# LCJebe/PCReg

Hardware: AMD Instinct MI355X
Metric: KNN Gpairs/s end-to-end (search + filters + RANSAC per step; registrations/s = 1000/ms_per_step) (higher is better)
Workload: dtype f32 (search: f16-split matrix-core candidates, exact f32 re-rank) / f64 (RANSAC)

## Files before the change

include/pcreg.h:

```cpp
#ifndef PCREG_H
#define PCREG_H
#include <stddef.h>
#include <stdint.h>

#ifdef __cplusplus
extern "C" {
#endif

#define PCREG_OK            0
#define PCREG_E_ARG         1
#define PCREG_E_HIP         2
#define PCREG_E_NODEVICE    3
#define PCREG_E_WORKSPACE   4

#define PCREG_KNN_MAX_K 32

#define PCREG_METRIC_SAD 0
#define PCREG_METRIC_SSD 1

typedef struct pcreg_ransac_opts {
    int32_t  minPtNum;
    int32_t  iterNum;
    double   thDist;
    double   thInlrRatio;
// ... 4 lines not shown

typedef struct pcreg_match_opts {
    int32_t metric;
    double  matchThreshold;
    double  maxRatio;
    int32_t unique;
    int32_t prenormalized;
    int32_t unnormalize;
    double  norm_factor;
    int32_t change_metric;
    double  metric_factor;
} pcreg_match_opts;

const char* pcreg_last_error(void);
const char* pcreg_version(void);
int  pcreg_device_count(int* count);
int  pcreg_set_device(int ordinal);
int  pcreg_device_name(char* buf, int cap);
int  pcreg_debug_set(const char* key, int value);
int  pcreg_debug_match_stats(long long out[8], int reset);
int  pcreg_debug_knn_stats(long long out[4], int reset);
int  pcreg_debug_knn_unit_stats(long long out[2], int reset);
int  pcreg_debug_ransac_stats(long long out[3], int reset);
int  pcreg_debug_cluster_stats(long long out[4], int reset);


int pcreg_estimate_transform(const double* pts1, const double* pts2, int n, int ld,
                             double T[16], int* empty);

int pcreg_calc_dists(const double T[16], const double* pts1, const double* pts2, int n, int ld,
                     double* d);

int pcreg_ransac(const double* pts1, const double* pts2, int n, int ld,
                 const pcreg_ransac_opts* opts, const int32_t* sample_idx,
                 double T[16], int32_t* inlier_idx, int* n_inliers, int* num_success,
                 int* max_inliers, int* failed, int32_t* iter_inl, int32_t* iter_inl_ref);

int pcreg_ransac_batched(const double* pts1, const double* pts2, int total, int ld,
                         const int32_t* offsets, int B, const pcreg_ransac_opts* opts,
                         const int32_t* sample_idx, double* T, int32_t* inlier_idx,
                         int32_t* n_inliers, int32_t* num_success, int32_t* max_inliers,
                         int32_t* failed);

int pcreg_knn2_points_f32(const float* q, int Q, int ldq, const float* m, int M, int ldm,
                          int32_t* idx, float* dist);

// ... 319 lines not shown
```

pcreg_amd/_lib.py:

```python
from __future__ import annotations

import ctypes as C
import os

_HERE = os.path.dirname(os.path.abspath(__file__))
LIB_PATH = os.environ.get("PCREG_LIB") or os.path.join(_HERE, "libpcreg_hip.so")

PCREG_OK, PCREG_E_ARG, PCREG_E_HIP, PCREG_E_NODEVICE, PCREG_E_WORKSPACE = 0, 1, 2, 3, 4
KNN_MAX_K = 32
METRIC_SAD, METRIC_SSD = 0, 1
LAYOUT_FEATURE_MAJOR, LAYOUT_ROW_MAJOR = 0, 1


class PcregError(RuntimeError):
    def __init__(self, code: int, msg: str):
        super().__init__(f"libpcreg_hip error {code}: {msg}")
        self.code = code


class RansacOpts(C.Structure):
    _fields_ = [("minPtNum", C.c_int32), ("iterNum", C.c_int32), ("thDist", C.c_double),
                ("thInlrRatio", C.c_double), ("REFINE", C.c_int32), ("VERBOSE", C.c_int32),
                ("seed", C.c_uint64)]


class MatchOpts(C.Structure):
    _fields_ = [("metric", C.c_int32), ("matchThreshold", C.c_double), ("maxRatio", C.c_double),
                ("unique", C.c_int32), ("prenormalized", C.c_int32), ("unnormalize", C.c_int32),
                ("norm_factor", C.c_double), ("change_metric", C.c_int32), ("metric_factor", C.c_double)]


class DescOpts(C.Structure):
    _fields_ = [("min_pts", C.c_int32), ("max_pts", C.c_int32), ("R", C.c_double), ("thVar", C.c_double * 2),
                ("k", C.c_double), ("ALIGN_POINTS", C.c_int32)]


class DevRansacResult(C.Structure):
    _fields_ = [("T", C.c_double * 16), ("n_inliers", C.c_int32), ("num_success", C.c_int32),
                ("max_inliers", C.c_int32), ("failed", C.c_int32), ("n", C.c_int32), ("winner", C.c_int32)]


SYMBOLS = [
    "pcreg_last_error", "pcreg_version", "pcreg_device_count", "pcreg_set_device", "pcreg_device_name", "pcreg_debug_set", "pcreg_debug_match_stats",
    "pcreg_debug_knn_stats", "pcreg_debug_knn_unit_stats", "pcreg_debug_ransac_stats", "pcreg_debug_cluster_stats", "pcreg_debug_dev_model_export", "pcreg_debug_search_export",
    "pcreg_estimate_transform", "pcreg_calc_dists", "pcreg_ransac", "pcreg_ransac_batched",
    "pcreg_knn2_points_f32", "pcreg_match_points_f32", "pcreg_match_features", "pcreg_get_matches", "pcreg_desc_set_create", "pcreg_desc_set_destroy", "pcreg_desc_set_size", "pcreg_get_matches_on_sets", "pcreg_get_matches_segmented_on_sets", "pcreg_sphere_counts", "pcreg_sphere_sweep", "pcreg_sphere_model_create", "pcreg_sphere_model_destroy", "pcreg_sphere_sweep_on_model", "pcreg_final_stage_limits", "pcreg_final_stage", "pcreg_get_matches_segmented", "pcreg_get_local_points",
    "pcreg_model_create", "pcreg_model_destroy", "pcreg_model_size", "pcreg_model_match_points_f32", "pcreg_model_knn_f32", "pcreg_knn_points_f32",
    "pcreg_model_range_f32", "pcreg_range_points_f32", "pcreg_model_cluster_f32", "pcreg_cluster_points_f32",
    "pcreg_dev_model_create", "pcreg_dev_model_destroy", "pcreg_dev_model_search_workspace", "pcreg_dev_model_search_f32",
    "pcreg_dev_model_knn_workspace", "pcreg_dev_model_knn_f32", "pcreg_dev_merge_topk_f32",
    "pcreg_dev_model_range_workspace", "pcreg_dev_model_range_count_f32", "pcreg_dev_model_range_fill_f32",
    "pcreg_dev_model_cluster_workspace", "pcreg_dev_model_cluster_f32",
    "pcreg_model_score_f32", "pcreg_dev_model_score_workspace", "pcreg_dev_model_score_f32",
    "pcreg_model_refit_f32", "pcreg_dev_model_refit_workspace", "pcreg_dev_model_refit_f32",
    "pcreg_model_normals_f32", "pcreg_point_normals_f32", "pcreg_dev_model_normals_workspace", "pcreg_dev_model_normals_f32",
    "pcreg_model_refit_plane_f32", "pcreg_dev_model_refit_plane_workspace", "pcreg_dev_model_refit_plane_f32",
    "pcreg_unique_rows3", "pcreg_aggregate_matches", "pcreg_dev_unique_rows3_workspace", "pcreg_dev_unique_rows3_f64",
    "pcreg_dev_aggregate_matches_workspace", "pcreg_dev_aggregate_matches", "pcreg_dev_estimate_transform_indexed",
    "pcreg_dev_model_match_f32", "pcreg_dev_model_match_table_f32", "pcreg_dev_match_from_table_f32",
    "pcreg_align_points_knn", "pcreg_align_points_knn_f32", "pcreg_align_points_knn_batched", "pcreg_spatial_histogram_descriptors",
    "pcreg_spatial_histogram_descriptors_f32", "pcreg_spatial_histogram_descriptors_mixed",
    "pcreg_dev_knn2_points_f32_workspace", "pcreg_dev_knn2_points_f32", "pcreg_dev_merge_top2_f32", "pcreg_dev_merge_top2_strided_f32",
    "pcreg_dev_ransac_workspace", "pcreg_dev_ransac",
    "pcreg_dev_ransac_partial", "pcreg_dev_ransac_finish", "pcreg_dev_ransac_finish_parts",
    "pcreg_dev_search_kernel_timing", "pcreg_dev_search_kernel_ms",
    "pcreg_dev_spatial_histogram_descriptors_workspace", "pcreg_dev_spatial_histogram_descriptors",
    "pcreg_dev_spatial_histogram_descriptors_rows_u16", "pcreg_dev_get_matches_rows_u16",
# ... 59 lines not shown
            vp, i, f = C.c_void_p, C.c_int, C.c_float
            L.pcreg_dev_model_refit_f32.argtypes = [vp, vp, i, i, vp, i, f, vp, vp, vp, vp, vp, vp, C.c_size_t, vp]
            L.pcreg_model_refit_f32.argtypes = [vp, vp, i, i, vp, i, f, i, vp, vp, vp, vp]
        if hasattr(L, "pcreg_dev_model_normals_workspace"):
            L.pcreg_dev_model_normals_workspace.restype = C.c_size_t
            L.pcreg_dev_model_normals_workspace.argtypes = [C.c_int] * 2
            vp, i = C.c_void_p, C.c_int
            L.pcreg_dev_model_normals_f32.argtypes = [vp, i, vp, vp, i, vp, vp, C.c_size_t, vp]
            L.pcreg_model_normals_f32.argtypes = [vp, i, vp, vp, i, vp]
            L.pcreg_point_normals_f32.argtypes = [vp, i, i, i, vp, vp, i, vp]
        if hasattr(L, "pcreg_dev_model_refit_plane_workspace"):
            L.pcreg_dev_model_refit_plane_workspace.restype = C.c_size_t
            L.pcreg_dev_model_refit_plane_workspace.argtypes = [C.c_int] * 3
            vp, i, f = C.c_void_p, C.c_int, C.c_float
            L.pcreg_dev_model_refit_plane_f32.argtypes = [vp, vp, i, i, vp, i, f, vp, i, vp, vp, vp, vp, vp, vp, vp, vp, C.c_size_t, vp]
            L.pcreg_model_refit_plane_f32.argtypes = [vp, vp, i, i, vp, i, f, i, vp, i, i, vp, vp, vp, vp, vp, vp]
        if hasattr(L, "pcreg_dev_unique_rows3_workspace"):
            for name in ("pcreg_dev_unique_rows3_workspace", "pcreg_dev_aggregate_matches_workspace"):
                getattr(L, name).restype = C.c_size_t
                getattr(L, name).argtypes = [C.c_int]
        for name, args in (("pcreg_debug_knn_stats", [C.POINTER(C.c_longlong), C.c_int]),
                           ("pcreg_debug_knn_unit_stats", [C.POINTER(C.c_longlong), C.c_int]),
                           ("pcreg_debug_ransac_stats", [C.POINTER(C.c_longlong), C.c_int]),
                           ("pcreg_debug_dev_model_export", [C.c_void_p] * 4 + [C.POINTER(C.c_float), C.c_void_p]),
                           ("pcreg_debug_search_export", [C.c_void_p, C.c_size_t, C.c_int, C.c_int] + [C.c_void_p] * 3)):
            if hasattr(L, name):
                getattr(L, name).argtypes = args
        _lib = L
    return _lib


def check(rc: int) -> None:
    if rc != PCREG_OK:
        raise PcregError(rc, lib().pcreg_last_error().decode(errors="replace"))
```

pcreg_amd/csrc/api.hip:

```cpp
#include "common.hpp"
#include <atomic>
#include <cstdarg>
#include <cmath>
#include <mutex>
#include <algorithm>
#include <vector>

namespace pcreg {

static thread_local char g_err[512] = "no error";
void set_error(const char* fmt, ...) {
    va_list ap; va_start(ap, fmt);
    vsnprintf(g_err, sizeof g_err, fmt, ap);
    va_end(ap);
}

constexpr int kKnnMaxK = PCREG_KNN_MAX_K;
constexpr int kKnnMaxQ = 4 << 20;
constexpr int kRangeMaxQ = 4 << 20;
constexpr int kScoreMaxQ = 4 << 20;
static std::mutex g_mu;
static int g_device_ok = -1;
static hipStream_t g_stream = nullptr;

// ... 30 lines not shown
        size[slot] = want;
    }
    *out = ptr[slot];
    return PCREG_OK;
}
void Scratch::release_all() {
    for (int i = 0; i < kSlots; ++i) if (ptr[i]) { (void)hipFree(ptr[i]); ptr[i] = nullptr; size[i] = 0; }
}
Scratch& scratch() { static Scratch s; return s; }

}

using namespace pcreg;

#define GUARD()                                                     \
    std::lock_guard<std::mutex> lock__(g_mu);                       \
    do { int rc__ = ensure_device(); if (rc__) return rc__; } while (0)
#define TRY(expr) do { int rc__ = (expr); if (rc__) return rc__; } while (0)

namespace pcreg {
static std::atomic<int> g_debug[kDbgCount];
int debug_flag(DebugKey k) { return g_debug[k].load(std::memory_order_relaxed); }
struct Counters { DebugKey key; int n; unsigned long long* dev; };
static Counters g_match_stats{kDbgMatchStats, 8, nullptr}, g_knn_stats{kDbgKnnStats, 6, nullptr}, g_ransac_stats{kDbgRansacStats, 3, nullptr},
                g_cluster_stats{kDbgClusterStats, 4, nullptr};
static unsigned long long* counters_dev(Counters& c) {
    if (!debug_flag(c.key)) return nullptr;
    if (!c.dev) {
        if (hipMalloc((void**)&c.dev, c.n * sizeof(unsigned long long)) != hipSuccess) { c.dev = nullptr; return nullptr; }
        (void)hipMemset(c.dev, 0, c.n * sizeof(unsigned long long));
    }
    return c.dev;
}
static int counters_read(const Counters& c, long long* out, int reset, int first = 0, int count = -1) {
    PCREG_ARG(out != nullptr);
    if (count < 0) count = c.n - first;
    for (int k = 0; k < count; ++k) out[k] = 0;
    if (!c.dev) return PCREG_OK;
    PCREG_HIP(hipDeviceSynchronize());
    unsigned long long h[8];
    PCREG_HIP(hipMemcpy(h, c.dev + first, count * sizeof h[0], hipMemcpyDeviceToHost));
    for (int k = 0; k < count; ++k) out[k] = (long long)h[k];
    if (reset) PCREG_HIP(hipMemset(c.dev + first, 0, count * sizeof h[0]));
    return PCREG_OK;
}
unsigned long long* match_stats_dev() { return counters_dev(g_match_stats); }
unsigned long long* knn_stats_dev() { return counters_dev(g_knn_stats); }
unsigned long long* ransac_stats_dev() { return counters_dev(g_ransac_stats); }
unsigned long long* cluster_stats_dev() { return counters_dev(g_cluster_stats); }
}

extern "C" {

int pcreg_debug_set(const char* key, int value) {
    static const char* const names[pcreg::kDbgCount] = {"knn_exact", "match_exact", "match_force_fallback", "ransac_fused", "ransac_nolane",
                                                        "ransac_f64score", "ransac_resident_f64", "align_times", "align_shape", "seg_debug",
                                                        "seg_batched", "seg_wave_finalize", "match_stats", "final_batch_mb", "knn_nocull",
                                                        "knn_stats", "ransac_pass2", "ransac_stats", "range_sort_cap", "cluster_noskip",
                                                        "cluster_stats", "knn_tail_cap", "score_batch_slots"};
    PCREG_ARG(key != nullptr);
    for (int k = 0; k < pcreg::kDbgCount; ++k)
        if (!strcmp(key, names[k])) { pcreg::g_debug[k].store(value, std::memory_order_relaxed); return PCREG_OK; }
    pcreg::set_error("pcreg_debug_set: unknown key '%s'", key);
    return PCREG_E_ARG;
}

int pcreg_debug_match_stats(long long out[8], int reset) { return pcreg::counters_read(pcreg::g_match_stats, out, reset); }
int pcreg_debug_knn_stats(long long out[4], int reset) { return pcreg::counters_read(pcreg::g_knn_stats, out, reset, 0, 4); }
int pcreg_debug_knn_unit_stats(long long out[2], int reset) { return pcreg::counters_read(pcreg::g_knn_stats, out, reset, 4, 2); }
int pcreg_debug_ransac_stats(long long out[3], int reset) { return pcreg::counters_read(pcreg::g_ransac_stats, out, reset); }
int pcreg_debug_cluster_stats(long long out[4], int reset) { return pcreg::counters_read(pcreg::g_cluster_stats, out, reset); }

const char* pcreg_last_error(void) { return g_err; }
const char* pcreg_version(void) { return "pcreg-hip 0.1 (gfx950)"; }

int pcreg_device_count(int* count) {
    PCREG_ARG(count != nullptr);
    hipError_t e = hipGetDeviceCount(count);
    if (e != hipSuccess) { *count = 0; (void)hipGetLastError(); }
    return PCREG_OK;
}

static void*  g_pin[2] = {nullptr, nullptr};
static size_t g_pin_bytes[2] = {0, 0};
static hipEvent_t g_pairs_ev = nullptr;

int pcreg_set_device(int ordinal) {
    std::lock_guard<std::mutex> lock(g_mu);
    int count = 0;
    if (hipGetDeviceCount(&count) != hipSuccess || count <= 0) { set_error("no HIP device available"); (void)hipGetLastError(); return PCREG_E_NODEVICE; }
    PCREG_ARG(ordinal >= 0 && ordinal < count);
    scratch().release_all();
    if (g_stream) { (void)hipStreamDestroy(g_stream); g_stream = nullptr; }
// ... 1855 lines not shown
```

pcreg_amd/csrc/common.hpp:

```cpp
#pragma once
#include <cstdlib>
#include <hip/hip_runtime.h>
#include <cstdint>
#include <cstdio>
#include <cstring>
#include <algorithm>
#include <string>
#include "../../include/pcreg.h"

namespace pcreg {

void set_error(const char* fmt, ...);
int  ensure_device();

#define PCREG_HIP(call)                                                                  \
    do {                                                                                 \
        hipError_t e__ = (call);                                                         \
        if (e__ != hipSuccess) {                                                         \
            ::pcreg::set_error("%s failed: %s (%s:%d)", #call, hipGetErrorString(e__),   \
                               __FILE__, __LINE__);                                      \
            return PCREG_E_HIP;                                                          \
        }                                                                                \
    } while (0)

// ... 28 lines not shown
    kDbgKnnExact = 0,
    kDbgMatchExact,
    kDbgMatchForceFallback,
    kDbgRansacFused,
    kDbgRansacNoLane,
    kDbgRansacF64Score,
    kDbgRansacResidentF64,
    kDbgAlignTimes,
    kDbgAlignShape,
    kDbgSegDebug,
    kDbgSegBatched,
    kDbgSegWaveFinalize,
    kDbgMatchStats,
    kDbgFinalBatchMB,
    kDbgKnnNoCull,
    kDbgKnnStats,
    kDbgRansacPass2,
    kDbgRansacStats,
    kDbgRangeSortCap,
    kDbgClusterNoSkip,
    kDbgClusterStats,
    kDbgKnnTailCap,
    kDbgScoreBatchSlots,
    kDbgCount
};
int debug_flag(DebugKey k);
unsigned long long* match_stats_dev();
unsigned long long* knn_stats_dev();
unsigned long long* ransac_stats_dev();
unsigned long long* cluster_stats_dev();
#ifdef PCREG_EXPERIMENTS
static inline int pcreg_env_int(const char* name, int dflt) { const char* e = getenv(name); return e ? atoi(e) : dflt; }
static inline const char* pcreg_env_str(const char* name) { return getenv(name); }
#define PCREG_EXP_ENV(name, dflt) pcreg_env_int(name, dflt)
#define PCREG_EXP_STR(name) pcreg_env_str(name)
#else
#define PCREG_EXP_ENV(name, dflt) (dflt)
#define PCREG_EXP_STR(name) ((const char*)nullptr)
#endif

static inline size_t align_up(size_t x, size_t a) { return (x + a - 1) / a * a; }

struct WsWalk {
    char* base; size_t off = 0;
    explicit WsWalk(void* b) : base((char*)b) {}
    void* take_bytes(size_t bytes) { void* p = base ? base + off : nullptr; off += bytes; return p; }
// ... 169 lines not shown
```

pcreg_amd/csrc/ransac.hip:

```cpp
#include "common.hpp"
#include "moments.hpp"
#include <cfloat>
#include <cstddef>
#include <cstdio>
#include <cstdlib>

namespace pcreg {
namespace {

constexpr int kBlock = 256;
constexpr int kWavesPerBlock = 4;
constexpr int HB = 4;

struct RansacArgs {
    const double* p1; const double* p2; int ld;
    const int32_t* offsets;
    const int32_t* n_dev;
    int n_cap; int iters; int m;
    double thDist; double ratio; int refine; unsigned long long seed;
    const int32_t* sample_idx;
    int hpw;
    int hyp0g;
    double* TF;
    int32_t* cnt1; int32_t* cnt2; unsigned char* has;
// ... 892 lines not shown
    double* T1; unsigned char* v1; unsigned char* pass1; unsigned char* v2;
    unsigned char* cert;
    double* certq;
    double* bounds;
    void* sel_ctr;
    double* bpart;
    int n_rec_blocks;
    double* mom;
    int32_t* part;
    int pb;
    unsigned long long* masks;
    int nslots_cap;
    double* rec;
    double* mpart;
    uint4* dig;
    int32_t* pass_list;
    int32_t* n_pass;
    unsigned char* dense;
    int use_lane;
    float* c32;
    int n32;
    float* T32a; float* T32b;
    int use_f32;
    float* p32;
    int32_t* perm;
    unsigned char* bkt;
    void* bctr;
};

__device__ __forceinline__ int staged_n(const RansacArgs& a) { return min(a.n_dev ? *a.n_dev : a.n_cap, a.n_cap); }
__device__ __forceinline__ void staged_origin(const StagedArgs& sa, double (&o)[6]) {
#pragma unroll
    for (int c = 0; c < 6; ++c) o[c] = sa.bounds[4 + c];
}

__device__ __forceinline__ void rs_records_body(const StagedArgs& sa, int block) {
    const RansacArgs& a = sa.a;
    const int n = staged_n(a);
    const int i = block * 256 + threadIdx.x;
    double m1 = 0.0, m2 = 0.0, c1m = 0.0, c2m = 0.0;
    double o[6] = {0.0, 0.0, 0.0, 0.0, 0.0, 0.0}, g2[2] = {0.0, 0.0};
    if (n >= 1) {
        const Pts<false> P0{a.p1, a.p2, a.ld, nullptr, n};
        ransac_origin(P0, n, o, g2);
        g2[0] *= kGridReach * kGridReach; g2[1] *= kGridReach * kGridReach;
        if (block == 0 && threadIdx.x < 8) {
// ... 227 lines not shown
            for (int s = 0; s < kSS; ++s) {
                const unsigned long long b = __ballot((sqdist(q[s], T) < th) & act[s]);
                cnt += __popcll(b);
                if (EMIT) {
                    asm volatile("v_writelane_b32 %0, %1, %2" : "+v"(mine_lo) : "s"((int)(unsigned)b), "n"(s));
                    asm volatile("v_writelane_b32 %0, %1, %2" : "+v"(mine_hi) : "s"((int)(unsigned)(b >> 32)), "n"(s));
                }
            }
            if (lane == 0) s_cnt[wave][h - h0] += cnt;
            if (EMIT && lane < kSS)
                sa.masks[(size_t)h * sa.nslots_cap + (size_t)pb * (kSPts / 64) + wave * kSS + lane] =
                    ((unsigned long long)(unsigned)mine_hi << 32) | (unsigned)mine_lo;
        }
    }
    __syncthreads();
    for (int hl = threadIdx.x; hl < h1 - h0; hl += kSW * 64) {
        int c = 0;
#pragma unroll
        for (int w = 0; w < kSW; ++w) c += s_cnt[w][hl];
        sa.part[(size_t)blockIdx.x * a.iters + h0 + hl] = c;
    }
}

__device__ __forceinline__ void make_t32(const double (&T)[12], const double (&o)[6], double A, double B, double th,
                                         float* __restrict__ out , const bool resident = false ) {
    const double u = 5.9604644775390625e-08;
    double rho = 0.0, tau = 0.0;
#pragma unroll
    for (int r = 0; r < 3; ++r) {
        const double tp = T[r * 4 + 3] + (T[r * 4] * o[3] + T[r * 4 + 1] * o[4] + T[r * 4 + 2] * o[5]) - o[r];
        rho = fmax(rho, sqrt(T[r * 4] * T[r * 4] + T[r * 4 + 1] * T[r * 4 + 1] + T[r * 4 + 2] * T[r * 4 + 2]));
        tau = fmax(tau, fabs(tp));
        out[r * 3] = (float)T[r * 4]; out[r * 3 + 1] = (float)T[r * 4 + 1]; out[r * 3 + 2] = (float)T[r * 4 + 2];
        out[9 + r] = (float)tp;
    }
    const double e1 = resident ? 6.1 * u * (A + B * rho + tau) : u * (A + 5.1 * (B * rho + tau));
    const double E = 1.5 * (2.0 * 1.7320508075688774 * sqrt(4.0 * th) * e1 + 3.0 * e1 * e1 + 5.2 * u * 4.0 * th);
    float lo = -INFINITY, hi = INFINITY;
    if (E == E && E <= 0.5 * th && th > 0.0 && tau < 1e30 && A < 1e15 && B < 1e15) {
        lo = (float)(th - E); if ((double)lo > th - E) lo = nextafterf(lo, -INFINITY);
        hi = (float)(th + E); if ((double)hi < th + E) hi = nextafterf(hi, INFINITY);
    }
    out[12] = lo; out[13] = hi; out[14] = 0.0f; out[15] = 0.0f;
}

__device__ __forceinline__ void rs_fold_maxima(const StagedArgs& sa, double (&mx)[4]) {
    __shared__ double s_mx[4][4];
#pragma unroll
    for (int k = 0; k < 4; ++k) mx[k] = 0.0;
    for (int b = threadIdx.x; b < sa.n_rec_blocks; b += 256) {
#pragma unroll
        for (int k = 0; k < 4; ++k) mx[k] = fmax(mx[k], sa.bpart[(size_t)b * 4 + k]);
    }
#pragma unroll
    for (int k = 0; k < 4; ++k) {
#pragma unroll
        for (int o_ = 32; o_ > 0; o_ >>= 1) mx[k] = fmax(mx[k], __shfl_xor(mx[k], o_));
    }
    if ((threadIdx.x & 63) == 0) {
#pragma unroll
        for (int k = 0; k < 4; ++k) s_mx[threadIdx.x >> 6][k] = mx[k];
    }
    __syncthreads();
#pragma unroll
    for (int k = 0; k < 4; ++k) mx[k] = fmax(fmax(s_mx[0][k], s_mx[1][k]), fmax(s_mx[2][k], s_mx[3][k]));
}
__device__ __forceinline__ void rs_digits_body(const StagedArgs& sa, uint4* __restrict__ dig, int block, const double (&bounds)[4]);
__global__ __launch_bounds__(256) void rs_stage2_kernel(StagedArgs sa, const double* __restrict__ TT, float* __restrict__ out, int n_t32,
                                                        uint4* __restrict__ dig) {
    const RansacArgs& a = sa.a;
    double mx[4];
    rs_fold_maxima(sa, mx);
    if ((int)blockIdx.x >= n_t32) { rs_digits_body(sa, dig, blockIdx.x - n_t32, mx); return; }
    if (blockIdx.x == 0 && threadIdx.x < 4) sa.bounds[threadIdx.x] = mx[threadIdx.x];
    const int h = blockIdx.x * blockDim.x + threadIdx.x;
    if (h >= a.iters || !sa.use_f32) return;
    const int n = staged_n(a);
    if (n < 1) return;
    double o[6]; staged_origin(sa, o);
    double T[12];
#pragma unroll
    for (int k = 0; k < 12; ++k) T[k] = TT[(size_t)h * 12 + k];
    make_t32(T, o, sqrt(mx[2]) * (1.0 + 1e-12), sqrt(mx[3]) * (1.0 + 1e-12), a.thDist, out + (size_t)h * 16);
}

__device__ __forceinline__ float sqdist32(const float (&p)[6], const float (&T)[12]) {
    const float tx = __builtin_fmaf(p[3], T[0], __builtin_fmaf(p[4], T[1], __builtin_fmaf(p[5], T[2], T[9])));
    const float ty = __builtin_fmaf(p[3], T[3], __builtin_fmaf(p[4], T[4], __builtin_fmaf(p[5], T[5], T[10])));
    const float tz = __builtin_fmaf(p[3], T[6], __builtin_fmaf(p[4], T[7], __builtin_fmaf(p[5], T[8], T[11])));
    const float dx = p[0] - tx, dy = p[1] - ty, dz = p[2] - tz;
    return __builtin_fmaf(dz, dz, __builtin_fmaf(dy, dy, dx * dx));
}

typedef int rs_i32x16 __attribute__((ext_vector_type(16)));
template <bool EMIT>
__global__ __launch_bounds__(kSW * 64) void rs_score32_kernel(StagedArgs sa, const double* __restrict__ TT,
                                                              const float* __restrict__ T32,
                                                              const unsigned char* __restrict__ valid,
                                                              int32_t* __restrict__ acc ) {
    const RansacArgs& a = sa.a;
    __shared__ int s_cnt[kSW][kSChunk];
    const int n = staged_n(a);
    const int lane = threadIdx.x & 63, wave = __builtin_amdgcn_readfirstlane(threadIdx.x >> 6);
    const int h0 = blockIdx.y * kSChunk, h1 = min(a.iters, h0 + kSChunk);
    const double th = a.thDist;
    for (int hl = threadIdx.x; hl < kSW * kSChunk; hl += kSW * 64) (&s_cnt[0][0])[hl] = 0;
    unsigned long long vmask[(kSChunk + 63) / 64];
#pragma unroll
    for (int k = 0; k < (kSChunk + 63) / 64; ++k) {
        const int h = h0 + k * 64 + lane;
        vmask[k] = __ballot(h < h1 && k * 64 + lane < kSChunk && valid[h] != 0);
    }
    __syncthreads();
    for (int pb = blockIdx.x; pb * kSPts < n; pb += gridDim.x) {
        float q[kSS][6];
        const int ibase = pb * kSPts + wave * kSS * 64 + lane;
#pragma unroll
        for (int s = 0; s < kSS; ++s) {
            const int i = ibase + s * 64;
            const bool act = i < n;
            const int ii = act ? i : 0;
#pragma unroll
            for (int c = 0; c < 6; ++c) q[s][c] = sa.c32[(size_t)c * sa.n32 + ii];
            if (!act) q[s][0] = __builtin_nanf("");
        }
        rs_i32x16 RA, RB;
#define PCREG_ROW_LOAD(R, H) { const float* rp_ = T32 + (size_t)min((H), h1 - 1) * 16; asm volatile("s_load_dwordx16 %0, %1, 0x0" : "=&s"(R) : "s"(rp_)); }
#define PCREG_ROW_WAIT(R) asm volatile("s_waitcnt lgkmcnt(0)" : "+s"(R))
#define PCREG_SCORE_HYP(H, R)                                                                                      \
        if ((vmask[((H) - h0) >> 6] >> (((H) - h0) & 63)) & 1ull) {                                \
            float T[12];                                                                                           \
            _Pragma("unroll") for (int k = 0; k < 12; ++k) { const int w_ = R[k]; T[k] = __int_as_float(w_); }                 \
            const int wlo_ = R[12], whi_ = R[13]; const float thlo = __int_as_float(wlo_), thhi = __int_as_float(whi_);          \
            unsigned long long b[kSS], band = 0ull;                                                                \
            _Pragma("unroll") for (int s = 0; s < kSS; ++s) {                                                      \
                const float d = sqdist32(q[s], T);                                                                 \
                b[s] = __ballot(d < thlo);                                                                         \
                band |= __ballot(d <= thhi) ^ b[s];       \
            }                                                                                                      \
            if (band != 0ull) {       \
                double T64[12];       \
                _Pragma("unroll") for (int k = 0; k < 12; ++k) T64[k] = TT[(size_t)(H) * 12 + k];    \
                _Pragma("unroll 1") for (int s = 0; s < kSS; ++s) {       \
                    const int i = ibase + s * 64;                         \
                    const bool act = i < n;                                                                        \
                    const int ii = act ? i : 0;                                                                    \
                    float qq[6];                                                                                   \
                    _Pragma("unroll") for (int c = 0; c < 6; ++c) qq[c] = sa.c32[(size_t)c * sa.n32 + ii];         \
                    if (!act) qq[0] = __builtin_nanf("");                                                          \
                    const float d = sqdist32(qq, T);                                                               \
                    if ((__ballot(d <= thhi) ^ __ballot(d < thlo)) != 0ull) {                     \
                        double p[6];                                                                               \
                        _Pragma("unroll") for (int c = 0; c < 3; ++c) { p[c] = a.p1[ii + (size_t)c * a.ld]; p[3 + c] = a.p2[ii + (size_t)c * a.ld]; } \
// ... 1033 lines not shown
                for (int e = 0; e < 15; ++e) mom[e] += pp[e];
            }
            v2 = fit_moments(c1, mom, o, T2, true);
        } else if (c1 == 3) {
#pragma unroll
            for (int e = 0; e < 27; ++e) mom[e] = sa.mom[(size_t)h * 27 + e];
            double A1[3][3], A2[3][3];
#pragma unroll
            for (int j = 0; j < 3; ++j)
#pragma unroll
                for (int c = 0; c < 3; ++c) { A1[j][c] = mom[j * 6 + c]; A2[j][c] = mom[j * 6 + 3 + c]; }
            v2 = fit_3pt(A1, A2, T2);
        } else {
#pragma unroll
            for (int e = 0; e < 27; ++e) mom[e] = sa.mom[(size_t)h * 27 + e];
            v2 = fit_moments(c1, mom, o, T2, sa.cert[h] != 0);
        }
    }
#pragma unroll
    for (int k = 0; k < 12; ++k) a.TF[(size_t)h * 12 + k] = T2[k];
    sa.v2[h] = v2;
    if (sa.use_f32 && v2) {
        double o32[6]; staged_origin(sa, o32);
        make_t32(T2, o32, sqrt(sa.bounds[2]) * (1.0 + 1e-12), sqrt(sa.bounds[3]) * (1.0 + 1e-12), a.thDist, sa.T32b + (size_t)h * 16);
    }
}

template <int NTHR>
__device__ void ransac_emit_result(const RansacArgs& a, int n, int off, pcreg_dev_ransac_result* r, int32_t* inlier_idx,
                                   bool failed, const double* s_T , int ns, int maxInl, int winner,
                                   int* s_base, int* s_wcnt) {
    const int lane = threadIdx.x & 63, wave = threadIdx.x >> 6;
    if (threadIdx.x == 0) *s_base = 0;
    __syncthreads();
    if (threadIdx.x < 16) {
        int k = threadIdx.x & 3, j = threadIdx.x >> 2;
        double v = 0.0;
        if (!failed) v = (j < 3) ? s_T[j * 4 + k] : (k == 3 ? 1.0 : 0.0);
        r->T[k + 4 * j] = v;
    }
    if (threadIdx.x == 0) {
        r->failed = failed; r->num_success = failed ? 0 : ns; r->max_inliers = failed ? 0 : maxInl;
        r->n = n; r->winner = winner;
    }
    if (failed) { if (threadIdx.x == 0) r->n_inliers = 0; return; }
    double T[12];
#pragma unroll
// ... 520 lines not shown
    s.cnt1 = w.take<int32_t>(h); s.cnt2 = w.take<int32_t>(h);
    s.has = w.take<unsigned char>(h); s.msc = w.take<double>(h * 16);
    sa.T1 = w.take<double>(h * 12); sa.mom = w.take<double>(h * 27);
    sa.part = w.take<int32_t>(h * kSMaxPB);
    sa.v1 = w.take<unsigned char>(h); sa.pass1 = w.take<unsigned char>(h); sa.v2 = w.take<unsigned char>(h);
    sa.cert = w.take<unsigned char>(h); sa.dense = w.take<unsigned char>(h);
    sa.bounds = (double*)w.take_bytes(256);
    sa.n_rec_blocks = (int)((slots * 64 + 255) / 256);
    sa.bpart = w.take<double>((size_t)sa.n_rec_blocks * 4);
    sa.sel_ctr = w.take_bytes(512);
    sa.certq = w.take<double>(h * 2);
    if (nc >= kStagedMinN) {
        sa.nslots_cap = (int)slots;
        sa.masks = w.take<unsigned long long>(h * slots);
        sa.rec = w.take<double>(slots * 64 * kRec + 32);
        sa.mpart = w.take<double>(staged_chunks_cap(nc) * h * 15);
        sa.pass_list = w.take<int32_t>(h);
        sa.dig = w.take<uint4>(slots * 2 * 256);
        sa.n_pass = (int32_t*)w.take_bytes(256);
        sa.n32 = (int)slots * 64;
        sa.c32 = w.take<float>((size_t)sa.n32 * 6);
        sa.T32a = w.take<float>(h * 16); sa.T32b = w.take<float>(h * 16);
        sa.p32 = w.take<float>((size_t)sa.n32 * 6);
        sa.perm = w.take<int32_t>((size_t)sa.n32);
        sa.bkt = w.take<unsigned char>((size_t)sa.n32);
        sa.bctr = w.take_bytes(align_up(sizeof(BCtr), 256));
    }
    *bytes = w.bytes(); return s;
}
size_t ransac_workspace_bytes(int iters, int B, int n_cap) { size_t b; (void)ransac_ws_layout(iters, B, n_cap, nullptr, &b); return b; }

constexpr int kHyp32NClasses = 2;
constexpr int kHyp32Classes[kHyp32NClasses] = {1024, 2048};
constexpr int kHyp32Waves[kHyp32NClasses] = {8, 16};
constexpr int kHyp32BatchCap = 3242;
static size_t hyp32_lds_bytes(int n, int nw) { return (size_t)((n + 127) / 128 * 128) * 72 + ((size_t)nw * 4 + 6) * sizeof(double); }
template <int NW>
static int launch_hyp32(const RansacArgs& a, dim3 grid, size_t lds, hipStream_t st) {
    static bool attr_set = false;
    if (!attr_set) {
        PCREG_HIP(hipFuncSetAttribute((const void*)ransac_hyp32_kernel<NW, true>, hipFuncAttributeMaxDynamicSharedMemorySize, 160 * 1024));
        PCREG_HIP(hipFuncSetAttribute((const void*)ransac_hyp32_kernel<NW, false>, hipFuncAttributeMaxDynamicSharedMemorySize, 160 * 1024));
        attr_set = true;
    }
    if (a.refine) hipLaunchKernelGGL((ransac_hyp32_kernel<NW, true>), grid, dim3(NW * 64), lds, st, a);
    else hipLaunchKernelGGL((ransac_hyp32_kernel<NW, false>), grid, dim3(NW * 64), lds, st, a);
// ... 28 lines not shown
        hipLaunchKernelGGL(ransac_hyp_kernel, dim3((o.iterNum + pb4 - 1) / pb4, B), dim3(kBlock), lds, st, a);
    } else if (n_cap > 0 && n_cap <= (offsets ? kHyp32BatchCap : kHyp32Classes[kHyp32NClasses - 1])) {
        int hpw = 64;
        while (hpw > 8 && total / hpw < 256LL * 4 * 2) hpw >>= 1;
        a.hpw = hpw;
        a.msc = lay.msc;
        const int c = n_cap <= kHyp32Classes[0] ? 0 : 1;
        a.n_lo = -1; a.n_hi = std::min(n_cap, kHyp32Classes[c]);
        const int nw = kHyp32Waves[c], per_block = hpw * nw;
        const dim3 grid((o.iterNum + per_block - 1) / per_block, B);
        const int rc = nw == 8 ? launch_hyp32<8>(a, grid, hyp32_lds_bytes(a.n_hi, nw), st) : launch_hyp32<16>(a, grid, hyp32_lds_bytes(a.n_hi, nw), st);
        if (rc != PCREG_OK) return rc;
        const int lo = a.n_hi;
        if (n_cap > lo) {
            a.n_lo = lo; a.n_hi = -1;
            const int pb4 = hpw * kWavesPerBlock;
            hipLaunchKernelGGL(ransac_hyp_kernel, dim3((o.iterNum + pb4 - 1) / pb4, B), dim3(kBlock), 0, st, a);
        }
    } else if (B == 1 && !offsets && staged_pays(n_cap, o.iterNum) && !debug_flag(kDbgRansacFused)) {
        StagedArgs sa = lay.sa;
        sel_ctr = sa.sel_ctr;
        sa.use_lane = a.refine && !debug_flag(kDbgRansacNoLane);
        sa.use_f32 = !debug_flag(kDbgRansacF64Score);
        int pb = (n_cap + kSPts - 1) / kSPts; if (pb > kSMaxPB) pb = kSMaxPB; if (pb < 1) pb = 1;
        sa.pb = pb;
        int hpw = (int)((total + 250LL * kTW - 1) / (250LL * kTW));
        if (hpw < 1) hpw = 1;
        if (hpw > 16) hpw = 16;
        a.hpw = hpw;
        sa.a = a;
        const int it = o.iterNum;
        const dim3 sgrid(pb, (it + kSChunk - 1) / kSChunk);
        const int n_fit = (it + 255) / 256;
        hipLaunchKernelGGL(rs_stage1_kernel, dim3((unsigned)(n_fit + sa.n_rec_blocks)), dim3(256), 0, st, sa, n_fit);
        const int n_t32 = (it + 255) / 256, n_dig = sa.use_lane ? (int)staged_slots_cap(n_cap) * 2 : 0;
        hipLaunchKernelGGL(rs_stage2_kernel, dim3((unsigned)(n_t32 + n_dig)), dim3(256), 0, st, sa, (const double*)sa.T1, sa.T32a, n_t32, sa.dig);
        if (sa.use_f32) {
            if (sa.use_lane)
                hipLaunchKernelGGL(rs_score32_kernel<true>, sgrid, dim3(kSW * 64), 0, st, sa, (const double*)sa.T1, (const float*)sa.T32a, (const unsigned char*)sa.v1, (int32_t*)nullptr);
            else
                hipLaunchKernelGGL(rs_score32_kernel<false>, sgrid, dim3(kSW * 64), 0, st, sa, (const double*)sa.T1, (const float*)sa.T32a, (const unsigned char*)sa.v1, (int32_t*)nullptr);
        } else if (sa.use_lane) {
            hipLaunchKernelGGL(rs_score_kernel<true>, sgrid, dim3(kSW * 64), 0, st, sa, (const double*)sa.T1, (const unsigned char*)sa.v1);
        } else {
            hipLaunchKernelGGL(rs_score_kernel<false>, sgrid, dim3(kSW * 64), 0, st, sa, (const double*)sa.T1, (const unsigned char*)sa.v1);
        }
        hipLaunchKernelGGL(rs_pass1_kernel, dim3((it + 255) / 256), dim3(256), 0, st, sa);
        if (a.refine) {
            if (sa.use_lane)
                hipLaunchKernelGGL(rs_moments_mfma_kernel, dim3((it + kMmWaves * kMmRows - 1) / (kMmWaves * kMmRows), (unsigned)staged_chunks_cap(n_cap)), dim3(kMmWaves * 64), 0, st, sa,
                                   (const uint4*)sa.dig, (const unsigned long long*)sa.masks);
            hipLaunchKernelGGL(rs_moments_kernel, dim3((it + hpw * kTW - 1) / (hpw * kTW)), dim3(kTBlock), 0, st, sa);
            hipLaunchKernelGGL(rs_fit2_kernel, dim3((it + 63) / 64), dim3(64), 0, st, sa);
            fold_finish = !part && n_cap <= kSelBlocks * kSelPerThread * kSelThreads;
            const int p2mode = debug_flag(kDbgRansacPass2);
            const bool bounded = fold_finish && sa.use_f32 && !iter_inl_ref && p2mode != 1 && (p2mode == 2 || bounded_pays(n_cap, it));
            if (bounded) {
                const int S = std::min(kBSeeds, it), nbc = (n_cap + kBBlk - 1) / kBBlk;
                const int n_seed_wg = (S * nbc + 3) / 4, n_ord_wg = (n_cap + 255) / 256;
// ... 132 lines not shown
```

Before: 122,200.

## Add slot-level certification to skip per-point RANSAC scoring behind debug flag

```diff
diff --git a/include/pcreg.h b/include/pcreg.h
--- a/include/pcreg.h
+++ b/include/pcreg.h
@@ -50,6 +50,7 @@
 int  pcreg_debug_knn_stats(long long out[4], int reset);
 int  pcreg_debug_knn_unit_stats(long long out[2], int reset);
 int  pcreg_debug_ransac_stats(long long out[3], int reset);
+int  pcreg_debug_ransac_slot_stats(long long out[2], int reset);
 int  pcreg_debug_cluster_stats(long long out[4], int reset);
 
 
diff --git a/pcreg_amd/_lib.py b/pcreg_amd/_lib.py
--- a/pcreg_amd/_lib.py
+++ b/pcreg_amd/_lib.py
@@ -42,7 +42,7 @@
 
 SYMBOLS = [
     "pcreg_last_error", "pcreg_version", "pcreg_device_count", "pcreg_set_device", "pcreg_device_name", "pcreg_debug_set", "pcreg_debug_match_stats",
-    "pcreg_debug_knn_stats", "pcreg_debug_knn_unit_stats", "pcreg_debug_ransac_stats", "pcreg_debug_cluster_stats", "pcreg_debug_dev_model_export", "pcreg_debug_search_export",
+    "pcreg_debug_knn_stats", "pcreg_debug_knn_unit_stats", "pcreg_debug_ransac_stats", "pcreg_debug_ransac_slot_stats", "pcreg_debug_cluster_stats", "pcreg_debug_dev_model_export", "pcreg_debug_search_export",
     "pcreg_estimate_transform", "pcreg_calc_dists", "pcreg_ransac", "pcreg_ransac_batched",
     "pcreg_knn2_points_f32", "pcreg_match_points_f32", "pcreg_match_features", "pcreg_get_matches", "pcreg_desc_set_create", "pcreg_desc_set_destroy", "pcreg_desc_set_size", "pcreg_get_matches_on_sets", "pcreg_get_matches_segmented_on_sets", "pcreg_sphere_counts", "pcreg_sphere_sweep", "pcreg_sphere_model_create", "pcreg_sphere_model_destroy", "pcreg_sphere_sweep_on_model", "pcreg_final_stage_limits", "pcreg_final_stage", "pcreg_get_matches_segmented", "pcreg_get_local_points",
     "pcreg_model_create", "pcreg_model_destroy", "pcreg_model_size", "pcreg_model_match_points_f32", "pcreg_model_knn_f32", "pcreg_knn_points_f32",
@@ -148,6 +148,7 @@
         for name, args in (("pcreg_debug_knn_stats", [C.POINTER(C.c_longlong), C.c_int]),
                            ("pcreg_debug_knn_unit_stats", [C.POINTER(C.c_longlong), C.c_int]),
                            ("pcreg_debug_ransac_stats", [C.POINTER(C.c_longlong), C.c_int]),
+                           ("pcreg_debug_ransac_slot_stats", [C.POINTER(C.c_longlong), C.c_int]),
                            ("pcreg_debug_dev_model_export", [C.c_void_p] * 4 + [C.POINTER(C.c_float), C.c_void_p]),
                            ("pcreg_debug_search_export", [C.c_void_p, C.c_size_t, C.c_int, C.c_int] + [C.c_void_p] * 3)):
             if hasattr(L, name):
diff --git a/pcreg_amd/csrc/api.hip b/pcreg_amd/csrc/api.hip
--- a/pcreg_amd/csrc/api.hip
+++ b/pcreg_amd/csrc/api.hip
@@ -76,7 +76,7 @@
 static std::atomic<int> g_debug[kDbgCount];
 int debug_flag(DebugKey k) { return g_debug[k].load(std::memory_order_relaxed); }
 struct Counters { DebugKey key; int n; unsigned long long* dev; };
-static Counters g_match_stats{kDbgMatchStats, 8, nullptr}, g_knn_stats{kDbgKnnStats, 6, nullptr}, g_ransac_stats{kDbgRansacStats, 3, nullptr},
+static Counters g_match_stats{kDbgMatchStats, 8, nullptr}, g_knn_stats{kDbgKnnStats, 6, nullptr}, g_ransac_stats{kDbgRansacStats, 5, nullptr},
                 g_cluster_stats{kDbgClusterStats, 4, nullptr};
 static unsigned long long* counters_dev(Counters& c) {
     if (!debug_flag(c.key)) return nullptr;
@@ -111,7 +111,7 @@
                                                         "ransac_f64score", "ransac_resident_f64", "align_times", "align_shape", "seg_debug",
                                                         "seg_batched", "seg_wave_finalize", "match_stats", "final_batch_mb", "knn_nocull",
                                                         "knn_stats", "ransac_pass2", "ransac_stats", "range_sort_cap", "cluster_noskip",
-                                                        "cluster_stats", "knn_tail_cap", "score_batch_slots"};
+                                                        "cluster_stats", "knn_tail_cap", "score_batch_slots", "ransac_slotcert"};
     PCREG_ARG(key != nullptr);
     for (int k = 0; k < pcreg::kDbgCount; ++k)
         if (!strcmp(key, names[k])) { pcreg::g_debug[k].store(value, std::memory_order_relaxed); return PCREG_OK; }
@@ -122,7 +122,8 @@
 int pcreg_debug_match_stats(long long out[8], int reset) { return pcreg::counters_read(pcreg::g_match_stats, out, reset); }
 int pcreg_debug_knn_stats(long long out[4], int reset) { return pcreg::counters_read(pcreg::g_knn_stats, out, reset, 0, 4); }
 int pcreg_debug_knn_unit_stats(long long out[2], int reset) { return pcreg::counters_read(pcreg::g_knn_stats, out, reset, 4, 2); }
-int pcreg_debug_ransac_stats(long long out[3], int reset) { return pcreg::counters_read(pcreg::g_ransac_stats, out, reset); }
+int pcreg_debug_ransac_stats(long long out[3], int reset) { return pcreg::counters_read(pcreg::g_ransac_stats, out, reset, 0, 3); }
+int pcreg_debug_ransac_slot_stats(long long out[2], int reset) { return pcreg::counters_read(pcreg::g_ransac_stats, out, reset, 3, 2); }
 int pcreg_debug_cluster_stats(long long out[4], int reset) { return pcreg::counters_read(pcreg::g_cluster_stats, out, reset); }
 
 const char* pcreg_last_error(void) { return g_err; }
diff --git a/pcreg_amd/csrc/common.hpp b/pcreg_amd/csrc/common.hpp
--- a/pcreg_amd/csrc/common.hpp
+++ b/pcreg_amd/csrc/common.hpp
@@ -74,6 +74,7 @@
     kDbgClusterStats,
     kDbgKnnTailCap,
     kDbgScoreBatchSlots,
+    kDbgRansacSlotCert,
     kDbgCount
 };
 int debug_flag(DebugKey k);
diff --git a/pcreg_amd/csrc/ransac.hip b/pcreg_amd/csrc/ransac.hip
--- a/pcreg_amd/csrc/ransac.hip
+++ b/pcreg_amd/csrc/ransac.hip
@@ -938,6 +938,9 @@
     int n32;
     float* T32a; float* T32b;
     int use_f32;
+    float* ssum;
+    int slotcert;
+    unsigned long long* cstats;
     float* p32;
     int32_t* perm;
     unsigned char* bkt;
@@ -1211,8 +1214,27 @@
     }
 }
 
+__device__ __forceinline__ void rs_cert_words(float* __restrict__ out , double rho, double tau, double A, double B, double th, float lo,
+                                              const float* R0 ) {
+    const double u = 5.9604644775390625e-08;
+    double d2 = 0.0;
+#pragma unroll
+    for (int k = 0; k < 9; ++k) { const double d = (double)out[k] - (double)R0[k]; d2 += d * d; }
+    const double dR = sqrt(d2) * (1.0 + 1e-12);
+    float f = (float)dR; if ((double)f < dR) f = nextafterf(f, INFINITY);
+    out[14] = f;
+    float sth = -INFINITY;
+    if (lo > 0.0f && th >= 1e-30) {
+        const double k18 = 3.814697265625e-06, ec = 2.0 * u * (A + 5.1 * (B * rho + tau));
+        const double sd = sqrt((double)lo) * (1.0 - k18) - 1.7320508075688774 * ec * (1.0 + k18);
+        if (sd > 0.0) { sth = (float)sd; if ((double)sth > sd) sth = nextafterf(sth, -INFINITY); }
+    }
+    out[15] = sth;
+}
+
 __device__ __forceinline__ void make_t32(const double (&T)[12], const double (&o)[6], double A, double B, double th,
-                                         float* __restrict__ out , const bool resident = false ) {
+                                         float* __restrict__ out , const bool resident = false ,
+                                         const float* R0 = nullptr , const bool cert = false) {
     const double u = 5.9604644775390625e-08;
     double rho = 0.0, tau = 0.0;
 #pragma unroll
@@ -1231,6 +1253,7 @@
         hi = (float)(th + E); if ((double)hi < th + E) hi = nextafterf(hi, INFINITY);
     }
     out[12] = lo; out[13] = hi; out[14] = 0.0f; out[15] = 0.0f;
+    if (cert) rs_cert_words(out, rho, tau, A, B, th, lo, R0);
 }
 
 __device__ __forceinline__ void rs_fold_maxima(const StagedArgs& sa, double (&mx)[4]) {
@@ -1255,6 +1278,102 @@
     for (int k = 0; k < 4; ++k) mx[k] = fmax(fmax(s_mx[0][k], s_mx[1][k]), fmax(s_mx[2][k], s_mx[3][k]));
 }
 __device__ __forceinline__ void rs_digits_body(const StagedArgs& sa, uint4* __restrict__ dig, int block, const double (&bounds)[4]);
+
+__device__ __forceinline__ void rs_anchor(const StagedArgs& sa, const double* __restrict__ TT, float (&R0)[9]) {
+    __shared__ float s_r0[9];
+    const int lane = threadIdx.x & 63, wave = threadIdx.x >> 6;
+    const bool ok = lane < sa.a.iters && sa.v1[lane] != 0;
+    const int m = __popcll(__ballot(ok));
+    float v[3];
+#pragma unroll
+    for (int k = 0; k < 3; ++k) {
+        const int e = min(wave + 4 * k, 8);
+        v[k] = ok ? (float)TT[(size_t)lane * 12 + (e / 3) * 4 + e % 3] : INFINITY;
+    }
+#pragma unroll
+    for (int k = 0; k < 3; ++k) {
+        const int e = wave + 4 * k;
+        if (e >= 9) break;
+        if (lane == 0) s_r0[e] = (e & 3) == 0 ? 1.0f : 0.0f;
+        int rank = 0;
+#pragma unroll
+        for (int j = 0; j < 64; ++j) {
+            const float w = __int_as_float(__builtin_amdgcn_readlane(__float_as_int(v[k]), j));
+            rank += (w < v[k] || (w == v[k] && j < lane)) ? 1 : 0;
+        }
+        if (ok && rank == (m - 1) / 2) s_r0[e] = v[k];
+    }
+    __syncthreads();
+#pragma unroll
+    for (int e = 0; e < 9; ++e) R0[e] = s_r0[e];
+}
+__device__ __forceinline__ void rs_slotsum_body(const StagedArgs& sa, int block, const float (&R0)[9]) {
+    const int lane = threadIdx.x & 63, slot = block * 4 + (threadIdx.x >> 6);
+    if (slot >= sa.nslots_cap) return;
+    const int n = staged_n(sa.a), i = slot * 64 + lane;
+    float* out = sa.ssum + (size_t)slot * 8;
+    if (slot * 64 + 64 > n) {
+        if (lane < 8) out[lane] = lane == 6 ? INFINITY : 0.0f;
+        return;
+    }
+    double q[6], c[6];
+#pragma unroll
+    for (int k = 0; k < 6; ++k) {
+        q[k] = (double)sa.c32[(size_t)k * sa.n32 + i];
+        double sum = q[k];
+#pragma unroll
+        for (int o_ = 32; o_ > 0; o_ >>= 1) sum += __shfl_xor(sum, o_);
+        c[k] = (double)(float)(sum * (1.0 / 64.0));
+    }
+    const double da[3] = {q[0] - c[0], q[1] - c[1], q[2] - c[2]}, db[3] = {q[3] - c[3], q[4] - c[4], q[5] - c[5]};
+    double e2 = 0.0, mag = 0.0;
+#pragma unroll
+    for (int r = 0; r < 3; ++r) {
+        const double r0 = (double)R0[r * 3], r1 = (double)R0[r * 3 + 1], r2 = (double)R0[r * 3 + 2];
+        const double e = da[r] - (r0 * db[0] + r1 * db[1] + r2 * db[2]);
+        e2 += e * e;
+        mag += fabs(da[r]) + fabs(r0 * db[0]) + fabs(r1 * db[1]) + fabs(r2 * db[2]);
+    }
+    double ei = sqrt(e2) * (1.0 + 1e-12) + 1e-14 * mag;
+    double bi = sqrt(db[0] * db[0] + db[1] * db[1] + db[2] * db[2]) * (1.0 + 1e-12);
+    if (!(ei < 1e300)) ei = INFINITY;
+    if (!(bi < 1e300)) ei = INFINITY;
+    if (!(bi < 1e300)) bi = INFINITY;
+#pragma unroll
+    for (int o_ = 32; o_ > 0; o_ >>= 1) { ei = fmax(ei, __shfl_xor(ei, o_)); bi = fmax(bi, __shfl_xor(bi, o_)); }
+    float ef = (float)ei; if ((double)ef < ei) ef = nextafterf(ef, INFINITY);
+    float bf = (float)bi; if ((double)bf < bi) bf = nextafterf(bf, INFINITY);
+    float v = 0.0f;
+#pragma unroll
+    for (int k = 0; k < 6; ++k) v = lane == k ? (float)c[k] : v;
+    v = lane == 6 ? ef : lane == 7 ? bf : v;
+    if (lane < 8) out[lane] = v;
+}
+__global__ __launch_bounds__(256) void rs_slotsum_kernel(StagedArgs sa, int n_sum) {
+    const RansacArgs& a = sa.a;
+    float R0[9];
+    rs_anchor(sa, sa.T1, R0);
+    if (blockIdx.x == 0 && threadIdx.x < 9) {
+        float v = 0.0f;
+#pragma unroll
+        for (int e = 0; e < 9; ++e) v = (int)threadIdx.x == e ? R0[e] : v;
+        sa.bounds[12 + threadIdx.x] = (double)v;
+    }
+    if ((int)blockIdx.x < n_sum) { rs_slotsum_body(sa, blockIdx.x, R0); return; }
+    const int h = (blockIdx.x - n_sum) * 256 + threadIdx.x;
+    if (h >= a.iters || staged_n(a) < 1) return;
+    double o[6]; staged_origin(sa, o);
+    double rho = 0.0, tau = 0.0;
+#pragma unroll
+    for (int r = 0; r < 3; ++r) {
+        const double* T = sa.T1 + (size_t)h * 12 + r * 4;
+        const double tp = T[3] + (T[0] * o[3] + T[1] * o[4] + T[2] * o[5]) - o[r];
+        rho = fmax(rho, sqrt(T[0] * T[0] + T[1] * T[1] + T[2] * T[2]));
+        tau = fmax(tau, fabs(tp));
+    }
+    float* row = sa.T32a + (size_t)h * 16;
+    rs_cert_words(row, rho, tau, sqrt(sa.bounds[2]) * (1.0 + 1e-12), sqrt(sa.bounds[3]) * (1.0 + 1e-12), a.thDist, row[12], R0);
+}
 __global__ __launch_bounds__(256) void rs_stage2_kernel(StagedArgs sa, const double* __restrict__ TT, float* __restrict__ out, int n_t32,
                                                         uint4* __restrict__ dig) {
     const RansacArgs& a = sa.a;
@@ -1283,7 +1402,7 @@
 
 typedef int rs_i32x16 __attribute__((ext_vector_type(16)));
 template <bool EMIT>
-__global__ __launch_bounds__(kSW * 64) void rs_score32_kernel(StagedArgs sa, const double* __restrict__ TT,
+__global__ __launch_bounds__(kSW * 64) __attribute__((amdgpu_waves_per_eu(6, 6))) void rs_score32_kernel(StagedArgs sa, const double* __restrict__ TT,
                                                               const float* __restrict__ T32,
                                                               const unsigned char* __restrict__ valid,
                                                               int32_t* __restrict__ acc ) {
@@ -1302,6 +1421,42 @@
     }
     __syncthreads();
     for (int pb = blockIdx.x; pb * kSPts < n; pb += gridDim.x) {
+        static_assert(kSS == 8 && kSChunk % 8 == 0 && kSChunk <= 64, "eight lanes per hypothesis, one mask word of hypotheses");
+        unsigned long long vrun = vmask[0];
+        if (sa.slotcert) {
+            const int slot0 = pb * (kSPts / 64) + wave * kSS;
+            const float4* sp = (const float4*)(sa.ssum + ((size_t)slot0 + (lane & 7)) * 8);
+            const float4 s0 = sp[0], s1 = sp[1];
+            int ncert = 0;
+#pragma unroll 1
+            for (int j = 0; j < kSChunk / 8; ++j) {
+                const int hl = j * 8 + (lane >> 3);
+                const bool ok = (vmask[0] >> hl) & 1ull;
+                const float4* rp = (const float4*)(T32 + (size_t)min(h0 + hl, h1 - 1) * 16);
+                const float4 r0 = rp[0], r1 = rp[1], r2 = rp[2], r3 = rp[3];
+                const float tx = __builtin_fmaf(s0.w, r0.x, __builtin_fmaf(s1.x, r0.y, __builtin_fmaf(s1.y, r0.z, r2.y)));
+                const float ty = __builtin_fmaf(s0.w, r0.w, __builtin_fmaf(s1.x, r1.x, __builtin_fmaf(s1.y, r1.y, r2.z)));
+                const float tz = __builtin_fmaf(s0.w, r1.z, __builtin_fmaf(s1.x, r1.w, __builtin_fmaf(s1.y, r2.x, r2.w)));
+                const float dx = s0.x - tx, dy = s0.y - ty, dz = s0.z - tz;
+                const float c2 = __builtin_fmaf(dz, dz, __builtin_fmaf(dy, dy, dx * dx));
+                const float g = r3.w - __builtin_fmaf(r3.z, s1.w, s1.z);
+                const unsigned long long cmj = __ballot(ok && g > 0.0f && c2 <= g * g);
+                ncert += __popcll(cmj);
+                const bool all8 = ((cmj >> (lane & 56)) & 0xFFull) == 0xFFull;
+                if (all8) {
+                    if ((lane & 7) == 0) s_cnt[wave][hl] += kSS * 64;
+                    if (EMIT) sa.masks[(size_t)(h0 + hl) * sa.nslots_cap + slot0 + (lane & 7)] = ~0ull;
+                }
+                const unsigned long long a8 = __ballot(all8 && (lane & 7) == 0);
+#pragma unroll
+                for (int g8 = 0; g8 < 8; ++g8) vrun &= ~(((a8 >> (8 * g8)) & 1ull) << (j * 8 + g8));
+            }
+            if (sa.cstats && lane == 0) {
+                const int sl = min(kSS, max(0, (n - (pb * kSPts + wave * kSS * 64) + 63) >> 6));
+                atomicAdd(sa.cstats, (unsigned long long)ncert);
+                atomicAdd(sa.cstats + 1, (unsigned long long)(__popcll(vmask[0]) * sl));
+            }
+        }
         float q[kSS][6];
         const int ibase = pb * kSPts + wave * kSS * 64 + lane;
 #pragma unroll
@@ -1317,7 +1472,7 @@
 #define PCREG_ROW_LOAD(R, H) { const float* rp_ = T32 + (size_t)min((H), h1 - 1) * 16; asm volatile("s_load_dwordx16 %0, %1, 0x0" : "=&s"(R) : "s"(rp_)); }
 #define PCREG_ROW_WAIT(R) asm volatile("s_waitcnt lgkmcnt(0)" : "+s"(R))
 #define PCREG_SCORE_HYP(H, R)                                                                                      \
-        if ((vmask[((H) - h0) >> 6] >> (((H) - h0) & 63)) & 1ull) {                                \
+        if ((vrun >> ((H) - h0)) & 1ull) {        \
             float T[12];                                                                                           \
             _Pragma("unroll") for (int k = 0; k < 12; ++k) { const int w_ = R[k]; T[k] = __int_as_float(w_); }                 \
             const int wlo_ = R[12], whi_ = R[13]; const float thlo = __int_as_float(wlo_), thhi = __int_as_float(whi_);          \
@@ -2397,7 +2552,11 @@
     sa.v2[h] = v2;
     if (sa.use_f32 && v2) {
         double o32[6]; staged_origin(sa, o32);
-        make_t32(T2, o32, sqrt(sa.bounds[2]) * (1.0 + 1e-12), sqrt(sa.bounds[3]) * (1.0 + 1e-12), a.thDist, sa.T32b + (size_t)h * 16);
+        float R0[9];
+#pragma unroll
+        for (int e = 0; e < 9; ++e) R0[e] = sa.slotcert ? (float)sa.bounds[12 + e] : 0.0f;
+        make_t32(T2, o32, sqrt(sa.bounds[2]) * (1.0 + 1e-12), sqrt(sa.bounds[3]) * (1.0 + 1e-12), a.thDist, sa.T32b + (size_t)h * 16, false,
+                 R0, sa.slotcert != 0);
     }
 }
 
@@ -2964,6 +3123,7 @@
         sa.c32 = w.take<float>((size_t)sa.n32 * 6);
         sa.T32a = w.take<float>(h * 16); sa.T32b = w.take<float>(h * 16);
         sa.p32 = w.take<float>((size_t)sa.n32 * 6);
+        sa.ssum = sa.p32;
         sa.perm = w.take<int32_t>((size_t)sa.n32);
         sa.bkt = w.take<unsigned char>((size_t)sa.n32);
         sa.bctr = w.take_bytes(align_up(sizeof(BCtr), 256));
@@ -3038,6 +3198,8 @@
         sel_ctr = sa.sel_ctr;
         sa.use_lane = a.refine && !debug_flag(kDbgRansacNoLane);
         sa.use_f32 = !debug_flag(kDbgRansacF64Score);
+        sa.slotcert = sa.use_f32 && debug_flag(kDbgRansacSlotCert) != 0;
+        { unsigned long long* cs = sa.slotcert ? ransac_stats_dev() : nullptr; sa.cstats = cs ? cs + 3 : nullptr; }
         int pb = (n_cap + kSPts - 1) / kSPts; if (pb > kSMaxPB) pb = kSMaxPB; if (pb < 1) pb = 1;
         sa.pb = pb;
         int hpw = (int)((total + 250LL * kTW - 1) / (250LL * kTW));
@@ -3051,6 +3213,10 @@
         hipLaunchKernelGGL(rs_stage1_kernel, dim3((unsigned)(n_fit + sa.n_rec_blocks)), dim3(256), 0, st, sa, n_fit);
         const int n_t32 = (it + 255) / 256, n_dig = sa.use_lane ? (int)staged_slots_cap(n_cap) * 2 : 0;
         hipLaunchKernelGGL(rs_stage2_kernel, dim3((unsigned)(n_t32 + n_dig)), dim3(256), 0, st, sa, (const double*)sa.T1, sa.T32a, n_t32, sa.dig);
+        if (sa.slotcert) {
+            const int n_sum = (sa.nslots_cap + 3) / 4;
+            hipLaunchKernelGGL(rs_slotsum_kernel, dim3((unsigned)(n_sum + n_t32)), dim3(256), 0, st, sa, n_sum);
+        }
         if (sa.use_f32) {
             if (sa.use_lane)
                 hipLaunchKernelGGL(rs_score32_kernel<true>, sgrid, dim3(kSW * 64), 0, st, sa, (const double*)sa.T1, (const float*)sa.T32a, (const unsigned char*)sa.v1, (int32_t*)nullptr);
```

Measured after the change: 122,100. About the same (-0.1%).
